# oneapi-src/ishmem

Hardware: AMD Instinct MI355X
Metric: GiB/s device-resident float32 sum-reduce at 1/2/4/8 PEs vs HBM+xGMI roofline (higher is better)
Workload: dtype f32

## Files before the change

### ishmem_amd/csrc/kernels.h

```cpp
#pragma once
#include <hip/hip_runtime.h>
#include <stddef.h>
#include <stdint.h>

#include "types.h"

namespace ishmemi {

constexpr int kMaxPes = 16;
constexpr int kMaxBlocks = 1024;
constexpr int kPhases = 4;
constexpr int kPhaseStart = 0, kPhaseMid = 1, kPhaseEnd = 2, kPhaseSync = 3;
constexpr size_t kFlagWordsPerTeam = (size_t) kPhases * kMaxBlocks * kMaxPes;
constexpr size_t kTeamFlagBytes = kFlagWordsPerTeam * 4 + 256;
constexpr int kBlock = 256;
constexpr int kUnroll = 4;
constexpr int kFaninBlock = 64;
constexpr int kFaninMaxGrid = (int) ((1ull << 31) / kFaninBlock);

constexpr int kEpWords = 16;
constexpr int kLineWords = 16;
constexpr int kEpReplicas = 64;
constexpr int kEpRepLine = 1, kEpShardLine = kEpRepLine + kEpReplicas, kEpShards = 8;
constexpr int kEpTopLine = kEpShardLine + kEpShards;
constexpr int kEpClaimLine = kEpTopLine + 1;
constexpr int kEpTeamWords = kEpClaimLine * kLineWords + kMaxBlocks;
constexpr int kEpEpoch = 0;
constexpr int kEpDone = 1;
constexpr int kEpRsHead = 2;
constexpr int kEpAgHead = 3;
constexpr int kEpStarted = 4;
constexpr int kEpFail = 5;
constexpr int kEpP1Done = 6;
struct ReduceArgs {
    const char *src[kMaxPes];
    const char *dstp[kMaxPes];
    char *dst;
    uint32_t *my_flags;
    uint32_t *peer_flags[kMaxPes];
    uint32_t *err;
    int *ret;
    uint64_t head;
    uint64_t nitems;
    uint64_t tail;
    uint64_t items_per_chunk;
    uint64_t seg_items;
    uint64_t timeout_ticks;
    int oneshot;
    uint32_t *ep_ctr;
    int p, me;
    uint64_t *trace;
};

#ifndef ISHMEMI_LL_TEAM_BYTES
#define ISHMEMI_LL_TEAM_BYTES (8u << 20)
#endif
constexpr size_t kLLTeamBytes = ISHMEMI_LL_TEAM_BYTES;
__host__ __device__ constexpr uint64_t ll_sender_granules(int p)
{
    return ((uint64_t) kLLTeamBytes / 8 / (2 * (uint64_t) (p < 1 ? 1 : p))) & ~uint64_t(127);
}
#ifndef ISHMEMI_LL_PAIRED
#define ISHMEMI_LL_PAIRED 0
#endif
__host__ __device__ constexpr uint64_t ll_granule(uint64_t item, int h)
{
// ... 67 lines not shown
constexpr int kRealignMaxGrid = (int) ((1ull << 31) / kRealignBlock);
#ifndef ISHMEMI_RS_REALIGN_BLOCK
#define ISHMEMI_RS_REALIGN_BLOCK 64
#endif
constexpr int kRsRealignBlock = ISHMEMI_RS_REALIGN_BLOCK;
#ifndef ISHMEMI_REALIGN_PEEL
#define ISHMEMI_REALIGN_PEEL 256
#endif
constexpr uint64_t kRealignPeel = ISHMEMI_REALIGN_PEEL;

struct FaninArgs {
    const char *src[kMaxFanin];
    char *dst;
    uint64_t head, nitems, tail;
    int nsrc;
    int realign;
    uint32_t shift[kMaxFanin];
    uint64_t total;
};

struct PhaseArgs {
    const char *src[kMaxPes];
    const char *dstp[kMaxPes];
    char *dst;
    uint64_t head, nitems, tail;
    uint64_t items_per_chunk;
    uint32_t elem;
    int p, me;
    int peer_nt;
    uint32_t shift;
    uint64_t total;
    int whole;
    int xcd_group;
};
hipError_t launch_rs_phase(int op, int dt, const PhaseArgs &a, hipStream_t s);
hipError_t launch_ag_phase(const PhaseArgs &a, hipStream_t s);

hipError_t launch_allreduce(int op, int dt, bool vec, const ReduceArgs &a, int grid,
                            hipStream_t s);
hipError_t launch_fanin(int op, int dt, bool vec, const FaninArgs &a, int grid, hipStream_t s);
hipError_t launch_team_sync(const ReduceArgs &a, hipStream_t s);
hipError_t launch_pull_probe(const FaninArgs &a, int policy, hipStream_t s);
void set_device_share(int share);
int device_share();
constexpr int kWaitSlotsDefault = 16;
void set_wait_slots(int slots);
int wait_slots();
void set_realign_grid_cap(int cap);
int realign_grid_cap();
void set_collect_realign(int on);
int collect_realign();
void set_phase_unaligned(int on);
int phase_unaligned();
hipError_t launch_occupy(int grid, uint64_t usec, hipStream_t s);
hipError_t launch_produce_u32(uint32_t *dst, const uint32_t *a, const uint32_t *b, uint64_t n, hipStream_t s);

struct RmaArgs {
    char *dst;
    const char *src;
    uint64_t head, nitems, tail;
};
hipError_t launch_rma_copy(const RmaArgs &a, bool put, int max_blocks, hipStream_t s);
hipError_t launch_read_all_u32(uint32_t *out, const uint32_t *p, uint64_t n, int grid, hipStream_t s);

}
```

### ishmem_amd/csrc/kernels_impl.h

```cpp
#pragma once
#include <algorithm>
#include <map>
#include <mutex>
#include <type_traits>

#include "kernels.h"

namespace ishmemi {
namespace {

constexpr int kSysCoherent = 17;
constexpr int kNonTemporal = 2;
constexpr uint64_t kTile = (uint64_t) kBlock * kUnroll;
#ifndef ISHMEMI_AR_OCC
#define ISHMEMI_AR_OCC 4
#endif


template <typename T>
struct alignas(16) Vec {
    T e[16 / sizeof(T)];
};

template <typename T>
// ... 786 lines not shown
    if (i0 + tid < a.nitems) wt_store(make_rsrc(uniform_ptr(a.dst + wo)), tid * 16u, acc);
}

template <typename T, int OP, int NS>
__global__ __launch_bounds__(kRealignBlock) void fanin_realign_kernel(FaninArgs a)
{
    static_assert(NS == 1 || NS == 2, "realigned fan-in: 1 or 2 sources");
    __shared__ u32x4 edge[NS][kRealignWaves + 1];
    const uint32_t tid = threadIdx.x;
    const uint64_t stride = (uint64_t) gridDim.x * kRealignBlock;
    const uint64_t first = (uint64_t) blockIdx.x * kRealignBlock;
    if (stride >= a.nitems) {
        if (first < a.nitems) fanin_realign_block<T, OP, NS>(a, edge, first);
    } else {
        for (uint64_t i0 = first; i0 < a.nitems; i0 += stride) {
            fanin_realign_block<T, OP, NS>(a, edge, i0);
            __syncthreads();
        }
    }
    if (blockIdx.x == 0) {
        const uint64_t tail_off = a.head + a.nitems * (16 / sizeof(T));
        for (int pass = 0; pass < 2; ++pass) {
            const uint64_t cnt = pass == 0 ? a.head : a.tail;
            for (uint64_t t = tid; t < cnt; t += kRealignBlock) {
                const uint64_t e = pass == 0 ? t : tail_off + t;
                T acc = ((const T *) a.src[0])[e];
                if constexpr (NS == 2) acc = op1<T, OP>(acc, ((const T *) a.src[1])[e]);
                ((T *) a.dst)[e] = acc;
            }
        }
    }
}

template <typename T, int OP, int P, bool NT, int R>
__device__ __forceinline__ void rs_phase_item(const PhaseArgs &a, uint64_t wb, bool valid)
{
    using Item = Vec<T>;
    const uint32_t off = threadIdx.x * 16u;
    Item x[P];
#pragma unroll
    for (int k = 0; k < P; ++k) {
        const int j = (R + k) % P;
        if (!valid) continue;
        if (NT || j == a.me) x[k] = bload<Item>(make_rsrc(uniform_ptr(a.src[j] + wb)), off);
        else x[k] = cload<Item>(make_rsrc(uniform_ptr(a.src[j] + wb)), off);
    }
    Item acc = x[(P - R) % P];
#pragma unroll
    for (int j = 1; j < P; ++j) acc = op1<T, OP>(acc, x[(j - R + P) % P]);
    if (valid) wt_store(make_rsrc(uniform_ptr(a.dst + wb)), off, acc);
}

template <typename T, int OP, int P, bool NT, int R = 0>
__device__ __forceinline__ void rs_phase_dispatch(const PhaseArgs &a, int rot, uint64_t wb, bool valid)
{
    if constexpr (R == P - 1) {
        rs_phase_item<T, OP, P, NT, R>(a, wb, valid);
    } else {
        if (rot == R) rs_phase_item<T, OP, P, NT, R>(a, wb, valid);
        else rs_phase_dispatch<T, OP, P, NT, R + 1>(a, rot, wb, valid);
    }
}

template <typename T, int OP>
__device__ __forceinline__ void rs_phase_item_any(const PhaseArgs &a, uint64_t wb, bool valid)
{
    using Item = Vec<T>;
    if (!valid) return;
    const uint32_t off = threadIdx.x * 16u;
    Item acc;
    for (int j = 0; j < a.p; ++j) {
        Item x;
        if (j == a.me || a.peer_nt) x = nt_load((const Item *) (a.src[j] + wb + off));
        else x = cload<Item>(make_rsrc(uniform_ptr(a.src[j] + wb)), off);
        acc = j == 0 ? x : op1<T, OP>(acc, x);
    }
    wt_store(make_rsrc(uniform_ptr(a.dst + wb)), off, acc);
}

template <typename T, int OP>
__device__ __forceinline__ void rs_phase_edges(const PhaseArgs &a)
{
    const int p = a.p, me = a.me;
    if (blockIdx.x == 0) {
        const int tid = threadIdx.x;
        const uint64_t tail_off = a.head + a.nitems * (16 / sizeof(T));
        for (int region = 0; region < 2; ++region) {
            const bool owner = a.whole || (region == 0 ? me == 0 : me == p - 1);
            const uint64_t cnt = region == 0 ? a.head : a.tail;
            if (!owner || (uint64_t) tid >= cnt) continue;
            const uint64_t rbase = (region == 0 ? 0 : tail_off) * sizeof(T);
            const uint32_t off = (uint32_t) (tid * sizeof(T));
            T acc = T();
            for (int j = 0; j < p; ++j) {
                T x;
                if (j == me) x = ((const T *) (a.src[j] + rbase))[tid];
                else x = cload<T>(make_rsrc(uniform_ptr(a.src[j] + rbase)), off);
                acc = (j == 0) ? x : op1<T, OP>(acc, x);
            }
            wt_store(make_rsrc(uniform_ptr(a.dst + rbase)), off, acc);
        }
    }
}

__device__ __forceinline__ uint64_t xcd_grouped_block(uint64_t b, uint64_t grid)
{
    if (b >= (grid & ~63ull)) return b;
    return (b & ~63ull) | ((b & 7) << 3) | ((b >> 3) & 7);
}

template <typename T, int OP, int P>
__global__ __launch_bounds__(kFaninBlock) void rs_phase_kernel(PhaseArgs a)
{
    const int me = a.me;
    const uint64_t cs = a.whole ? 0 : min((uint64_t) me * a.items_per_chunk, a.nitems);
    const uint64_t ce = a.whole ? a.nitems : min(cs + a.items_per_chunk, a.nitems);
    const uint64_t head_bytes = a.head * sizeof(T);
    const uint64_t stride = (uint64_t) gridDim.x * kFaninBlock;
    const uint64_t blk = a.shift && a.xcd_group ? xcd_grouped_block(blockIdx.x, gridDim.x) : blockIdx.x;
    auto body = [&](auto nt) {
        for (uint64_t i0 = cs + blk * kFaninBlock; i0 < ce; i0 += stride) {
            const bool valid = i0 + threadIdx.x < ce;
            const uint64_t wb = head_bytes + i0 * 16;
            if constexpr (P > 0) rs_phase_dispatch<T, OP, P, decltype(nt)::value>(a, (int) ((i0 / kFaninBlock) % P), wb, valid);
            else rs_phase_item_any<T, OP>(a, wb, valid);
        }
    };
    if (a.peer_nt) {
        body(std::true_type{});
    } else {
        body(std::false_type{});
    }
    rs_phase_edges<T, OP>(a);
}

template <typename T, int OP, int BS, int G>
__device__ __forceinline__ void rs_realign_block(const PhaseArgs &a, u32x4 (*edge)[BS / 64 + 1], uint64_t i0, uint64_t ce)
{
    const int p = a.p, me = a.me;
    const uint32_t tid = threadIdx.x;
    const uint64_t wb = a.head * sizeof(T) + i0 * 16;
    Vec<T> acc;
    for (int g0 = 0; g0 < p; g0 += G) {
        if (g0) __syncthreads();
        u32x4 A[G], B[G];
#pragma unroll
        for (int k = 0; k < G; ++k) {
            const int j = g0 + k;
            if (j >= p) break;
            if (j == me || a.peer_nt) realign_issue<kNonTemporal, BS>(a.src[j], a.shift, a.total, wb, edge[k], A[k], B[k]);
            else realign_issue<kSysCoherent, BS>(a.src[j], a.shift, a.total, wb, edge[k], A[k], B[k]);
        }
        __syncthreads();
#pragma unroll
        for (int k = 0; k < G; ++k) {
            const int j = g0 + k;
            if (j >= p) break;
            const Vec<T> x = __builtin_bit_cast(Vec<T>, realign_finish(edge[k], A[k], B[k], a.shift));
            acc = j == 0 ? x : op1<T, OP>(acc, x);
        }
    }
    if (i0 + tid < ce) wt_store(make_rsrc(uniform_ptr(a.dst + wb)), tid * 16u, acc);
}

template <typename T, int OP>
__global__ __launch_bounds__(kRsRealignBlock) void rs_phase_realign_kernel(PhaseArgs a)
{
    constexpr int BS = kRsRealignBlock, G = 4;
    __shared__ u32x4 edge[G][BS / 64 + 1];
    const uint64_t cs = a.whole ? 0 : min((uint64_t) a.me * a.items_per_chunk, a.nitems);
    const uint64_t ce = a.whole ? a.nitems : min(cs + a.items_per_chunk, a.nitems);
    const uint64_t stride = (uint64_t) gridDim.x * BS;
    const uint64_t first = cs + (uint64_t) blockIdx.x * BS;
    if (cs + stride >= ce) {
        if (first < ce) rs_realign_block<T, OP, BS, G>(a, edge, first, ce);
    } else {
        for (uint64_t i0 = first; i0 < ce; i0 += stride) {
            rs_realign_block<T, OP, BS, G>(a, edge, i0, ce);
            __syncthreads();
        }
    }
    rs_phase_edges<T, OP>(a);
}

__global__ __launch_bounds__(kFaninBlock) void ag_phase_kernel(PhaseArgs a)
{
    const int p = a.p, me = a.me;
    const uint64_t head_bytes = a.head * a.elem;
    const uint64_t peers = (uint64_t) (p - 1);
    const uint64_t blocks = (a.items_per_chunk + kFaninBlock - 1) / kFaninBlock;
    const uint64_t work = peers * blocks;
    const uint32_t off = threadIdx.x * 16u;
    for (uint64_t w = blockIdx.x; w < work; w += gridDim.x) {
        const int j = (me + 1 + (int) (w % peers)) % p;
        const uint64_t js = min((uint64_t) j * a.items_per_chunk, a.nitems);
        const uint64_t je = min(js + a.items_per_chunk, a.nitems);
        const uint64_t i0 = js + (w / peers) * kFaninBlock;
        if (i0 + threadIdx.x < je) {
            const uint64_t wb = head_bytes + i0 * 16;
            const u32x4 x = a.peer_nt ? nt_load((const u32x4 *) (a.dstp[j] + wb + off))
                                      : cload<u32x4>(make_rsrc(uniform_ptr(a.dstp[j] + wb)), off);
            wt_store(make_rsrc(uniform_ptr(a.dst + wb)), off, x);
        }
    }
    if (blockIdx.x == 0) {
        const uint32_t tid = threadIdx.x;
        const uint64_t tail_b = (uint64_t) a.tail * a.elem;
        const uint64_t tail_base = head_bytes + a.nitems * 16;
        if (me != 0 && tid < head_bytes)
            a.dst[tid] = (char) cload<uint8_t>(make_rsrc(uniform_ptr(a.dstp[0])), tid);
        if (me != p - 1 && tid < tail_b)
            a.dst[tail_base + tid] = (char) cload<uint8_t>(make_rsrc(uniform_ptr(a.dstp[p - 1] + tail_base)), tid);
    }
}

template <typename K>
int phase_grid(K, uint64_t items)
{
    const uint64_t g = (items + kFaninBlock - 1) / kFaninBlock;
    return (int) std::max<uint64_t>(1, std::min<uint64_t>(g, (uint64_t) kFaninMaxGrid));
}

template <typename T, int OP>
hipError_t rs_phase_t(const PhaseArgs &a, hipStream_t s)
{
    const uint64_t cs = a.whole ? 0 : std::min((uint64_t) a.me * a.items_per_chunk, a.nitems);
    const uint64_t len = a.whole ? a.nitems : std::min(cs + a.items_per_chunk, a.nitems) - cs;
    auto go = [&](auto kernel) {
        hipLaunchKernelGGL(kernel, dim3(phase_grid(kernel, len)), dim3(kFaninBlock), 0, s, a);
    };
    if (a.shift && !phase_unaligned()) {
        uint64_t g = std::max<uint64_t>(1, std::min<uint64_t>((len + kRsRealignBlock - 1) / kRsRealignBlock,
                                                              (1ull << 31) / kRsRealignBlock));
        if (realign_grid_cap() > 0) g = std::min<uint64_t>(g, (uint64_t) realign_grid_cap());
        hipLaunchKernelGGL((rs_phase_realign_kernel<T, OP>), dim3((unsigned) g), dim3(kRsRealignBlock), 0, s, a);
    } else if (a.p == 2) go(rs_phase_kernel<T, OP, 2>);
    else if (a.p == 4) go(rs_phase_kernel<T, OP, 4>);
    else if (a.p == 8) go(rs_phase_kernel<T, OP, 8>);
    else go(rs_phase_kernel<T, OP, 0>);
    return hipGetLastError();
}

template <typename T, int OP>
__device__ __forceinline__ uint64_t fold8(uint64_t acc, uint64_t x)
{
    constexpr int K = 8 / sizeof(T);
    struct alignas(8) W {
        T e[K];
    };
    W a = __builtin_bit_cast(W, acc), b = __builtin_bit_cast(W, x);
#pragma unroll
    for (int i = 0; i < K; ++i) a.e[i] = op1<T, OP>(a.e[i], b.e[i]);
    return __builtin_bit_cast(uint64_t, a);
}

__device__ __forceinline__ uint64_t ll_load(const char *p, uint64_t valid)
{
    if (valid == 8) {
        if (((uintptr_t) p & 7) == 0) return *(const uint64_t *) p;
        if (((uintptr_t) p & 3) == 0)
            return (uint64_t) ((const uint32_t *) p)[0] | ((uint64_t) ((const uint32_t *) p)[1] << 32);
    }
    uint64_t mine = 0;
    for (uint32_t k = 0; k < (uint32_t) valid; ++k) mine |= (uint64_t) (uint8_t) p[k] << (8 * k);
    return mine;
}

__device__ __forceinline__ void ll_store(char *p, uint64_t valid, uint64_t v)
// ... 59 lines not shown
                        __hip_atomic_fetch_or(a.err, 1u << 4, __ATOMIC_RELAXED, __HIP_MEMORY_SCOPE_SYSTEM);
                        break;
                    }
                    __builtin_amdgcn_s_sleep(1);
                }
                x = (h0 & 0xffffffffull) | (h1 << 32);
            }
            if (a.mode == kLLCollect || a2a) ll_store(a.dst + (uint64_t) j * a.nbytes + off, valid, x);
            else if (bcast) { if (j == a.root) ll_store(a.dst + off, valid, x); }
            else if (j <= last) acc = (j == 0) ? x : fold8<T, OP>(acc, x);
        }
        if (ok && a.mode != kLLCollect && !a2a && !bcast) ll_store(a.dst + off, valid, acc);
    }
    if (!ok && a.ret) __hip_atomic_fetch_or(a.ret, 1, __ATOMIC_RELAXED, __HIP_MEMORY_SCOPE_SYSTEM);
    kernel_epoch_done(a, ep);
}

inline int resident_blocks_of(const void *kernel);

template <typename T, int OP>
hipError_t ll_t(const LLArgs &a, hipStream_t s)
{
    const uint64_t nitems = (a.nbytes + 7) / 8;
    const uint64_t want = std::max<uint64_t>(1, (nitems + kBlock - 1) / kBlock);
    const int grid = (int) std::min<uint64_t>(want, (uint64_t) resident_blocks_of((const void *) ll_kernel<T, OP>));
    hipLaunchKernelGGL((ll_kernel<T, OP>), dim3(grid), dim3(kBlock), 0, s, a);
    return hipGetLastError();
}

__global__ __launch_bounds__(kBlock) void team_sync_kernel(ReduceArgs a)
{
    const uint32_t ep = kernel_epoch(a);
    const bool ok = pe_barrier(a, ep, kPhaseSync, 0);
    if (threadIdx.x == 0 && !ok && a.ret)
        __hip_atomic_fetch_or(a.ret, 1, __ATOMIC_RELAXED, __HIP_MEMORY_SCOPE_SYSTEM);
    kernel_epoch_done(a, ep);
}

template <int OP, typename S, typename U>
using Canon = std::conditional_t<(OP == ISHMEMI_OP_MAX || OP == ISHMEMI_OP_MIN), S, U>;

inline int resident_blocks_of(const void *kernel)
{
    static std::mutex mu;
    static std::map<const void *, int> cache;
    static int cus = 0;
    std::lock_guard<std::mutex> lk(mu);
    if (cus <= 0) {
        int dev = 0;
        (void) hipGetDevice(&dev);
        if (hipDeviceGetAttribute(&cus, hipDeviceAttributeMultiprocessorCount, dev) != hipSuccess) {
            (void) hipGetLastError();
            cus = 1;
        }
    }
    int per = 0;
    auto it = cache.find(kernel);
    if (it != cache.end()) {
        per = it->second;
    } else {
        if (hipOccupancyMaxActiveBlocksPerMultiprocessor(&per, kernel, kBlock, 0) != hipSuccess) {
            (void) hipGetLastError();
            per = 1;
        }
        per = std::max(per, 1);
        cache[kernel] = per;
    }
    const long long slots = (long long) device_share() * wait_slots();
// ... 97 lines not shown
```

### ishmem_amd/csrc/runtime.cpp

```cpp
#include <hip/hip_runtime.h>
#include <stdio.h>
#include <stdlib.h>
#include <string.h>
#include <strings.h>
#include <stdint.h>
#include <errno.h>
#include <sys/prctl.h>
#include <unistd.h>

#include <algorithm>
#include <chrono>
#include <limits>
#include <map>
#include <mutex>
#include <string>
#include <vector>

#include "bootstrap.h"
#include "kernels.h"
#include "types.h"

namespace ishmemi {
namespace {

// ... 181 lines not shown
long long wait_slots_floor() { return std::max<long long>(1, env_ll("GPU_MAX_HW_QUEUES", 4)); }

struct Team {
    bool valid = false;
    int start = 0, stride = 1, size = 1;
    int my_idx = -1;
    int num_contexts = 0;
    bool colocated = true;
};

struct TeamMem {
    uint32_t *flags[kMaxPes] = {};
    uint64_t *ring[kMaxPes] = {};
    int pool_idx = -1;
    char *fold_scratch = nullptr;
    size_t fold_scratch_bytes = 0;
};

struct PoolBlock {
    uint32_t *ptr = nullptr;
    hipIpcMemHandle_t handle{};
    bool in_use = false;
};

constexpr long long kPhasedOff = std::numeric_limits<long long>::max();
constexpr long long kPhasedDefault = 4ll << 20;

struct PeRecord {
    int32_t pe, pid, device, flags_kind;
    int32_t flags_kind_requested;
    char pci_bus[32];
    uint64_t heap_size;
    int64_t max_blocks, ll_max_bytes, oneshot_p2, phased_min;
    uint64_t staging_bytes;
    int64_t staging_slots;
    int64_t xgmi_ll_max, xgmi_fold_max;
    hipIpcMemHandle_t heap_handle;
    hipIpcMemHandle_t flags_handle;
};

struct State {
    std::mutex mu;
    bool initialized = false;
    int pe = 0, npes = 1, device = 0;
    ShmBootstrap boot;

    char *heap = nullptr;
    size_t heap_size = 0;
    std::map<size_t, size_t> free_list;
    std::map<size_t, size_t> used;
    char *peer_heap[kMaxPes] = {};

    uint32_t *flags = nullptr;
    int flags_kind = 0;
    uint32_t *peer_flags[kMaxPes] = {};
    int dev_id[kMaxPes] = {};
    TeamMem tmem[kMaxTeams];
    int teams_max = kTeamsMaxDefault;
    size_t team_block_bytes = 0;
    std::vector<PoolBlock> team_pool;
    std::map<std::pair<int, uint32_t>, void *> peer_pool;
    uint32_t *err_host = nullptr;
    uint32_t *err_dev = nullptr;
    uint64_t *exch_host = nullptr, *exch_dev = nullptr;
    uint32_t *done_host = nullptr, *done_dev = nullptr;
    uint32_t done_seq = 0;
    int block_spin = 2;
    ishmemi_c_device_ctx_t *dctx = nullptr;
    uint32_t *dev_epochs = nullptr;
    uint32_t *kern_ep = nullptr;

    char *team_scratch = nullptr;
    char *count_slots = nullptr;
    char *staging = nullptr;
    size_t staging_bytes = 0;
    hipStream_t copy_in = nullptr, copy_out = nullptr;
    hipStream_t rma_stream = nullptr;
    hipEvent_t rma_ev = nullptr;
    bool rma_pending = false;
    hipStream_t last_stream = nullptr;
    bool last_stream_set = false;
    bool stream_order = false;
    long long oneshot_p2 = 32ll << 20;
    long long phased_min = kPhasedDefault;
    hipEvent_t order_ev = nullptr;
    hipEvent_t staging_ev = nullptr;
    bool staging_used = false;
    int staging_slots = kStagingSlotsDefault;
    int staged_copy_kernel = 0;
    bool test_flags_unavailable = false;
    int phased_peer_nt = 0;
    int ar_shifted = 1;
    int rs_xcd = 1;
    int direct_p2 = 1;
    int direct_max_pes = 4;
    int direct_inplace = 1;
    long long xgmi_ll_max = -1, xgmi_fold_max = -1;
    double xgmi_link_bps = 76.8e9;
    hipEvent_t ev_in[kMaxStagingSlots] = {}, ev_red[kMaxStagingSlots] = {}, ev_out[kMaxStagingSlots] = {};

    Team teams[kMaxTeams];
    int max_blocks = kMaxBlocks;
    long long ll_max_bytes = (long long) kLLDefaultBytes;
    long long timeout_ms = 60000;
    int debug = 0;
    int error_count = 0;
    uint64_t *trace = nullptr;
    bool phase_events = false, phase_recorded = false;
    hipEvent_t phase_ev[6] = {};
    double init_us[8] = {};
};

const char *const kInitPhase[8] = {"hip", "heap", "flags", "bootstrap", "ipc_heap", "ipc_flags", "teams", "total"};

State &S()
{
    static State s;
    return s;
}

struct CtxSlots {
    std::mutex mu;
    std::vector<const void *> shadows;
};
// ... 406 lines not shown
    a.ret = ret;
    a.trace = s.trace;
    const void *srcs[1] = {src};
    Plan pl = make_plan(dst, srcs, 1, n, es, t.size, s.max_blocks, 0);
    a.head = pl.head;
    a.nitems = pl.nitems;
    a.tail = pl.tail;
    a.items_per_chunk = pl.items_per_chunk;
    a.seg_items = pl.seg_items;
    const uintptr_t d0 = (uintptr_t) dst, s0 = (uintptr_t) src, nb = n * es;
    const bool realign = !pl.vec && d0 % es == 0 && s0 % es == 0 && nb >= kRealignMinBytes;
    if (realign && (long long) nb < s.phased_min && s.ar_shifted) {
        const void *dsts[1] = {dst};
        pl = make_plan(dst, dsts, 1, n, es, t.size, s.max_blocks, 0);
        a.head = pl.head;
        a.nitems = pl.nitems;
        a.tail = pl.tail;
        a.items_per_chunk = pl.items_per_chunk;
        a.seg_items = pl.seg_items;
    }
    const bool disjoint = d0 + nb <= s0 || s0 + nb <= d0;
    const PathLimits lim = team_limits(s, t);
    const bool fold_size = lim.fold > 0 && (long long) nb <= lim.fold;
    char *scratch = nullptr;
    if (fold_size && d0 == s0 && pl.vec && s.direct_inplace && (uint64_t) t.size * nb <= kInplaceFoldBytes) {
        const TeamMem &m = s.tmem[team];
        if (!m.fold_scratch || m.fold_scratch_bytes < nb + 16)
            return fail("reduce: the team's in-place fold scratch is missing");
        scratch = m.fold_scratch + (d0 & 15);
    }
    const bool inplace_fold = scratch != nullptr;
    const bool direct = (fold_size && disjoint && (pl.vec || realign)) || inplace_fold;
    if ((pl.vec || realign) && (direct || (long long) nb >= s.phased_min)) {
        PhaseArgs ph;
        memset(&ph, 0, sizeof(ph));
        for (int j = 0; j < t.size; ++j) {
            ph.src[j] = a.src[j];
            ph.dstp[j] = a.dstp[j];
        }
        ph.dst = a.dst;
        ph.head = pl.head;
        ph.nitems = pl.nitems;
        ph.tail = pl.tail;
        ph.items_per_chunk = pl.items_per_chunk;
        ph.elem = (uint32_t) es;
        ph.p = t.size;
        ph.me = t.my_idx;
        ph.peer_nt = s.phased_peer_nt;
        ph.whole = direct ? 1 : 0;
        ph.xcd_group = s.rs_xcd && device_share() == 1 ? 1 : 0;
        if (inplace_fold) ph.dst = scratch;
        if (realign) {
            const uint64_t h = std::min<uint64_t>(n, ((16 - d0 % 16) % 16) / es);
            ph.head = h;
            ph.nitems = (n - h) * es / 16;
            ph.tail = n - h - ph.nitems * (16 / es);
            ph.items_per_chunk = items_per_chunk(ph.nitems, t.size);
            ph.shift = (uint32_t) ((s0 + h * es) % 16);
            ph.total = nb;
        }
        const bool ev = s.phase_events && !capturing(st);
        auto mark = [&](int k) -> int {
            if (ev) HIP_TRY(hipEventRecord(s.phase_ev[k], st));
            return 0;
        };
        if (mark(0)) return 1;
        if (team_barrier(s, team, a, st)) return 1;
        if (mark(1)) return 1;
        HIP_TRY(launch_rs_phase(op, dt, ph, st));
        if (mark(2)) return 1;
        if (!direct) {
            if (team_barrier(s, team, a, st)) return 1;
            if (mark(3)) return 1;
            HIP_TRY(launch_ag_phase(ph, st));
        } else if (mark(3)) {
            return 1;
        }
        if (mark(4)) return 1;
        if (team_barrier(s, team, a, st)) return 1;
        if (mark(5)) return 1;
        if (inplace_fold && launch_copy(dst, scratch, nb, st)) return 1;
        s.phase_recorded = s.phase_recorded || ev;
        return 0;
    }
    if (t.size == 2 && (long long) nb <= lim.oneshot && disjoint) {
        a.oneshot = 1;
        a.items_per_chunk = pl.nitems;
        a.seg_items = seg_items(pl.nitems);
        pl.grid = (int) std::max<uint64_t>(
            1, std::min<uint64_t>(nsegs(pl.nitems, a.seg_items), (uint64_t) s.max_blocks));
    }
    HIP_TRY(launch_allreduce(op, dt, pl.vec, a, pl.grid, st));
    return 0;
}

constexpr size_t kPinMinBytes = (size_t) 1 << 20;

bool pageable_host(const void *p)
{
    hipPointerAttribute_t attr;
    if (hipPointerGetAttributes(&attr, p) != hipSuccess) {
        (void) hipGetLastError();
        return true;
    }
// ... 746 lines not shown
    if (env_flag_false("ISHMEM_ENABLE_GPU_IPC") && g_env_error.empty())
        g_env_error = std::string("ISHMEM_ENABLE_GPU_IPC=") + getenv("ISHMEM_ENABLE_GPU_IPC") +
                      " is not supported: ishmem_amd's collectives are IPC-only (peer loads over xGMI from "
                      "IPC-mapped heaps; there is no proxy path)";
    if (env_flag_true("ISHMEM_ENABLE_ACCESSIBLE_HOST_HEAP") && g_env_error.empty())
        g_env_error = std::string("ISHMEM_ENABLE_ACCESSIBLE_HOST_HEAP=") + getenv("ISHMEM_ENABLE_ACCESSIBLE_HOST_HEAP") +
                      " is not supported: the symmetric heap is device memory shared over IPC (host buffers "
                      "are accepted by every call and staged)";
    s.max_blocks = (int) std::min<long long>(kMaxBlocks, std::max<long long>(1, env_ll("ISHMEM_MAX_BLOCKS", kMaxBlocks)));
    s.timeout_ms = std::max<long long>(1, env_ll("ISHMEM_TIMEOUT_MS", 60000));
    s.ll_max_bytes = std::min<long long>((long long) kLLMaxBytes,
                                         std::max<long long>(0, env_bytes("ISHMEM_LL_MAX_BYTES", (long long) kLLDefaultBytes)));
    s.debug = debug_level();
    s.trace = nullptr;
    s.stream_order = env_ll("ISHMEM_STREAM_ORDER", 0) != 0;
    s.oneshot_p2 = std::max<long long>(0, env_bytes("ISHMEM_ONESHOT_P2_MAX_BYTES", 32ll << 20));
    s.phased_min = env_bytes("ISHMEM_PHASED_MIN_BYTES", kPhasedDefault);
    if (s.phased_min < 0) s.phased_min = kPhasedOff;
    s.staging_bytes = (env_size("ISHMEM_STAGING_SIZE", (size_t) 128 << 20) + kHeapAlign - 1) &
                      ~(size_t) (kHeapAlign - 1);
    s.staging_slots = (int) std::min<long long>(kMaxStagingSlots, std::max<long long>(2, env_ll("ISHMEM_STAGING_SLOTS", kStagingSlotsDefault)));
    s.staged_copy_kernel = (int) (env_ll("ISHMEM_STAGED_COPY_KERNEL", kStagedCopyKernelDefault) & 3);
    const size_t heap_request = env_size("ISHMEM_SYMMETRIC_SIZE", (size_t) 4 << 30);
    const int first_kind = (int) std::min<long long>(kFlagsCoarse, std::max<long long>(0, env_ll("ISHMEM_FLAGS_KIND", 0)));
#ifdef ISHMEMI_TEST_HOOKS
    s.test_flags_unavailable = env_ll("ISHMEM_TEST_FLAGS_UNAVAILABLE", 0) != 0;
#else
    for (const char *hook : {"ISHMEM_TEST_FLAGS_UNAVAILABLE", "ISHMEM_TEST_PCI_BUS"})
        if (getenv(hook) && g_env_error.empty())
            g_env_error = std::string(hook) + " is a test hook, honoured only by libishmem_amd_testhooks.so";
#endif
    const bool ep_uncached = env_ll("ISHMEM_EP_UNCACHED", 0) != 0;
    s.phased_peer_nt = env_ll("ISHMEM_PHASED_PEER_NT", 0) != 0;
    s.teams_max = kTeamsMaxDefault;
    if (const char *tm = getenv("ISHMEM_TEAMS_MAX"); tm && *tm) {
        const long long v = env_ll("ISHMEM_TEAMS_MAX", kTeamsMaxDefault);
        if (v < 0 && g_env_error.empty())
            g_env_error = std::string("ISHMEM_TEAMS_MAX='") + tm + "' is not a team count";
        else if (v > kMaxTeams && g_env_error.empty())
            g_env_error = "ISHMEM_TEAMS_MAX=" + std::to_string(v) + ": requested " + std::to_string(v) +
                          " teams, but only " + std::to_string(kMaxTeams) + " are supported";
        s.teams_max = (int) std::min<long long>(kMaxTeams, std::max<long long>(kPredefTeams, v));
    }
    s.xgmi_ll_max = std::max<long long>(-1, env_bytes("ISHMEM_XGMI_LL_MAX_BYTES", -1));
    s.xgmi_fold_max = std::max<long long>(-1, env_bytes("ISHMEM_XGMI_FOLD_MAX_BYTES", -1));
    s.xgmi_link_bps = 76.8e9;
    if (const char *bk = getenv("ISHMEM_BARRIER_KIND"); bk && *bk && strcasecmp(bk, "kernel") != 0 && g_env_error.empty())
        g_env_error = std::string("ISHMEM_BARRIER_KIND='") + bk +
                      "' is not supported: team barriers are the one-workgroup barrier kernel ('kernel')";
    if (!g_env_error.empty()) {
        const std::string e = g_env_error;
        g_env_error.clear();
        return fail("init: " + e);
    }
    warn_unknown_env();

    using clk = std::chrono::steady_clock;
    const auto t_start = clk::now();
    auto t_mark = t_start;
    auto phase_done = [&](int k) {
        const auto now = clk::now();
        s.init_us[k] = std::chrono::duration<double, std::micro>(now - t_mark).count();
        t_mark = now;
        if (s.debug > 1) {
            fprintf(stderr, "[ishmem_amd] PE %d init: %s done (%.1f ms)\n", pe, kInitPhase[k], s.init_us[k] / 1000.0);
            fflush(stderr);
// ... 32 lines not shown
    s.done_host = (uint32_t *) ((char *) s.err_host + kErrDoneOffset);
    s.done_dev = (uint32_t *) ((char *) s.err_dev + kErrDoneOffset);
    s.done_seq = 0;
    HIP_TRY(hipDeviceSynchronize());

    for (int i = 0; i < kMaxPes; ++i) {
        s.peer_heap[i] = nullptr;
        s.peer_flags[i] = nullptr;
    }
    s.peer_heap[pe] = s.heap;
    s.peer_flags[pe] = s.flags;
    for (int i = 0; i < kMaxPes; ++i) s.dev_id[i] = 0;
    phase_done(2);

    if (npes > 1) {
        struct PtracerWindow {
            PtracerWindow() { prctl(PR_SET_PTRACER, PR_SET_PTRACER_ANY, 0, 0, 0); }
            ~PtracerWindow() { prctl(PR_SET_PTRACER, 0, 0, 0, 0); }
        } ptracer_window;
        std::string err;
        if (s.boot.attach(pe, npes, key, (int) std::max<long long>(s.timeout_ms, 10000), err))
            return fail(err);
        PeRecord mine{};
        mine.pe = pe;
        mine.pid = (int32_t) getpid();
        mine.device = s.device;
        mine.flags_kind = s.flags_kind;
        mine.flags_kind_requested = first_kind;
        mine.heap_size = s.heap_size;
        mine.max_blocks = s.max_blocks;
        mine.ll_max_bytes = s.ll_max_bytes;
        mine.oneshot_p2 = s.oneshot_p2;
        mine.phased_min = s.phased_min;
        mine.staging_bytes = s.staging_bytes;
        mine.staging_slots = s.staging_slots;
        mine.xgmi_ll_max = s.xgmi_ll_max;
        mine.xgmi_fold_max = s.xgmi_fold_max;
        if (hipDeviceGetPCIBusId(mine.pci_bus, sizeof(mine.pci_bus), s.device) != hipSuccess) {
            (void) hipGetLastError();
            snprintf(mine.pci_bus, sizeof(mine.pci_bus), "dev%d", s.device);
        }
#ifdef ISHMEMI_TEST_HOOKS
        if (const char *fake = getenv("ISHMEM_TEST_PCI_BUS"))
            snprintf(mine.pci_bus, sizeof(mine.pci_bus), "%s", fake);
#endif
        if (hipError_t e = hipIpcGetMemHandle(&mine.heap_handle, s.heap); e != hipSuccess)
            return fail(std::string("init: hipIpcGetMemHandle of the symmetric heap: ") + hipGetErrorString(e) + ipc_hint());
        mine.flags_handle = flags_handle;
        PeRecord all[kMaxPes];
        if (s.boot.allgather(&mine, all, sizeof(PeRecord), err)) return fail(err);
        phase_done(3);
        for (int j = 0; j < npes; ++j) {
            s.ll_max_bytes = std::min<long long>(s.ll_max_bytes, all[j].ll_max_bytes);
            s.oneshot_p2 = std::min<long long>(s.oneshot_p2, all[j].oneshot_p2);
            s.phased_min = std::max<long long>(s.phased_min, all[j].phased_min);
            s.staging_bytes = std::min<size_t>(s.staging_bytes, all[j].staging_bytes);
            s.staging_slots = (int) std::min<int64_t>(s.staging_slots, all[j].staging_slots);
            if (all[j].xgmi_ll_max >= 0)
                s.xgmi_ll_max = s.xgmi_ll_max < 0 ? all[j].xgmi_ll_max : std::min<long long>(s.xgmi_ll_max, all[j].xgmi_ll_max);
            if (all[j].xgmi_fold_max >= 0)
                s.xgmi_fold_max = s.xgmi_fold_max < 0 ? all[j].xgmi_fold_max
                                                       : std::min<long long>(s.xgmi_fold_max, all[j].xgmi_fold_max);
        }
        int share = 0;
        for (int j = 0; j < npes; ++j)
            share += strncmp(all[j].pci_bus, mine.pci_bus, sizeof(mine.pci_bus)) == 0;
        for (int j = 0; j < npes; ++j) {
            s.dev_id[j] = j;
            for (int k = 0; k < j; ++k)
                if (strncmp(all[j].pci_bus, all[k].pci_bus, sizeof(all[j].pci_bus)) == 0) {
                    s.dev_id[j] = s.dev_id[k];
                    break;
                }
        }
        bool coarse_forced = false;
        for (int j = 0; j < npes; ++j) coarse_forced = coarse_forced || all[j].flags_kind_requested == kFlagsCoarse;
        set_device_share(share);
        for (int j = 0; j < npes; ++j) {
            if (j == pe) continue;
            if (all[j].heap_size != s.heap_size)
                return fail("init: ISHMEM_SYMMETRIC_SIZE differs between PEs");
            if (all[j].device != s.device) {
                int can = 0;
                if (hipDeviceCanAccessPeer(&can, s.device, all[j].device) != hipSuccess || !can)
                    return fail("init: no peer access from device " + std::to_string(s.device) +
                                " to device " + std::to_string(all[j].device) + " (PE " +
                                std::to_string(j) + ")");
                hipError_t e = hipDeviceEnablePeerAccess(all[j].device, 0);
// ... 1209 lines not shown

const char *ishmemi_c_last_error(void) { return g_last_error.c_str(); }

int ishmemi_c_phase_times(float *ms5)
{
    State &s = S();
    if (!ms5) return fail("phase_times: null output");
    if (!s.phase_recorded || !s.phase_ev[0]) return fail("phase_times: no phased reduce recorded (set_param phase_events 1)");
    HIP_TRY(hipEventSynchronize(s.phase_ev[5]));
    for (int k = 0; k < 5; ++k) HIP_TRY(hipEventElapsedTime(&ms5[k], s.phase_ev[k], s.phase_ev[k + 1]));
    return 0;
}

int ishmemi_c_set_param(const char *name, long long value)
{
    State &s = S();
    std::lock_guard<std::mutex> lk(s.mu);
    const std::string n = name ? name : "";
    if (n == "max_blocks") s.max_blocks = (int) std::min<long long>(kMaxBlocks, std::max<long long>(1, value));
    else if (n == "staged_copy_kernel") s.staged_copy_kernel = (int) (value & 3);
    else if (n == "wait_slots") {
        if (value < wait_slots_floor())
            return fail("set_param: wait_slots " + std::to_string(value) + " is below " +
                        std::to_string(wait_slots_floor()) + " (GPU_MAX_HW_QUEUES), see ISHMEM_WAIT_SLOTS");
        set_wait_slots((int) std::min<long long>(1 << 20, value));
    }
    else if (n == "timeout_ms") s.timeout_ms = std::max<long long>(1, value);
    else if (n == "stream_order") s.stream_order = value != 0;
    else if (n == "oneshot_p2_max_bytes") s.oneshot_p2 = std::max<long long>(0, value);
    else if (n == "phased_min_bytes") s.phased_min = value < 0 ? kPhasedOff : value;
    else if (n == "ll_max_bytes") s.ll_max_bytes = std::min<long long>((long long) kLLMaxBytes, std::max<long long>(0, value));
    else if (n == "debug") s.debug = (int) value;
    else if (n == "phased_peer_nt") s.phased_peer_nt = value != 0;
    else if (n == "xgmi_ll_max_bytes") s.xgmi_ll_max = std::max<long long>(-1, value);
    else if (n == "xgmi_fold_max_bytes") s.xgmi_fold_max = std::max<long long>(-1, value);
    else if (n == "xgmi_link_mbps") {
        if (value <= 0) return fail("set_param: xgmi_link_mbps must be positive");
        s.xgmi_link_bps = (double) value * 1e6;
    }
    else if (n == "realign_grid_cap") set_realign_grid_cap((int) std::min<long long>(std::max<long long>(value, 0), 1 << 30));
    else if (n == "collect_realign") set_collect_realign((int) (value != 0));
    else if (n == "ar_shifted") s.ar_shifted = value != 0;
    else if (n == "rs_xcd") s.rs_xcd = value != 0;
    else if (n == "direct_p2") s.direct_p2 = value != 0;
    else if (n == "direct_inplace") s.direct_inplace = value != 0;
    else if (n == "block_spin") s.block_spin = (int) std::min<long long>(std::max<long long>(value, 0), 2);
    else if (n == "direct_max_pes") s.direct_max_pes = (int) std::min<long long>(std::max<long long>(value, 2), kMaxPes);
    else if (n == "phase_unaligned") set_phase_unaligned((int) (value != 0));
    else if (n == "trace_buffer") s.trace = (uint64_t *) (uintptr_t) value;
    else if (n == "phase_events") {
        if (value && !s.phase_ev[0])
            for (hipEvent_t &e : s.phase_ev) HIP_TRY(hipEventCreate(&e));
        s.phase_events = value != 0;
    }
    else return fail("set_param: unknown parameter " + n);
    return 0;
}

long long ishmemi_c_get_param(const char *name)
{
    State &s = S();
    const std::string n = name ? name : "";
    if (n == "max_blocks") return s.max_blocks;
    if (n == "staged_copy_kernel") return s.staged_copy_kernel;
    if (n == "wait_slots") return wait_slots();
    if (n == "timeout_ms") return s.timeout_ms;
    if (n == "stream_order") return s.stream_order ? 1 : 0;
    if (n == "oneshot_p2_max_bytes") return s.oneshot_p2;
    if (n == "phased_min_bytes") return s.phased_min == kPhasedOff ? -1 : s.phased_min;
    if (n == "ll_max_bytes") return s.ll_max_bytes;
    if (n == "ll_capacity_bytes") return (long long) ll_capacity(s.npes);
    if (n == "ll_limit_bytes") return team_limits(s, s.teams[0]).ll;
    if (n == "fold_limit_bytes") return team_limits(s, s.teams[0]).fold;
    if (n == "team_colocated") return s.teams[0].colocated ? 1 : 0;
    if (n == "xgmi_ll_max_bytes") return s.xgmi_ll_max;
    if (n == "xgmi_fold_max_bytes") return s.xgmi_fold_max;
    if (n == "xgmi_link_mbps") return (long long) (s.xgmi_link_bps / 1e6);
    if (n == "teams_max") return s.teams_max;
    if (n == "flag_block_bytes") return s.initialized ? (long long) (kBaseAllocBytes + s.team_block_bytes) : 0;
    if (n == "flag_block_pool_bytes") return (long long) (s.team_pool.size() * kTeamAllocBytes);
    if (n == "flag_block_bytes_round5") return (long long) kRound5FlagBytes;
    for (int k = 0; k < 8; ++k)
        if (n == std::string("init_us_") + kInitPhase[k]) return (long long) s.init_us[k];
    if (n == "debug") return s.debug;
    if (n == "phased_peer_nt") return s.phased_peer_nt;
    if (n == "realign_grid_cap") return realign_grid_cap();
    if (n == "collect_realign") return collect_realign();
    if (n == "ar_shifted") return s.ar_shifted;
    if (n == "rs_xcd") return s.rs_xcd;
    if (n == "direct_p2") return s.direct_p2;
    if (n == "direct_inplace") return s.direct_inplace;
    if (n == "block_spin") return s.block_spin;
    if (n == "direct_max_pes") return s.direct_max_pes;
    if (n == "phase_unaligned") return phase_unaligned();
    if (n == "flags_fine_grained") return s.flags_kind != kFlagsCoarse ? 1 : 0;
    if (n == "flags_kind") return s.flags_kind;
    if (n == "staging_bytes") return (long long) s.staging_bytes;
    if (n == "staging_slots") return s.staging_slots;
    if (n == "heap_bytes") return (long long) s.heap_size;
    if (n == "device_share") return device_share();
    if (n == "launch_words") return (long long) (uintptr_t) s.kern_ep;
    if (n == "cu_count") {
        int dev = 0, cus = 0;
        if (hipGetDevice(&dev) != hipSuccess ||
            hipDeviceGetAttribute(&cus, hipDeviceAttributeMultiprocessorCount, dev) != hipSuccess) {
            (void) hipGetLastError();
            return -1;
        }
        return cus;
    }
    return -1;
}

int ishmemi_c_error_count(void)
{
    State &s = S();
    int pending = 0;
    if (s.err_host)
// ... 46 lines not shown
```

Measured before the change: 3136.

## Push reduced chunks directly to all peers, fusing reduce-scatter with all-gather

In the phased allreduce path, the reduce-scatter kernel can now write each reduced chunk to every peer's destination buffer, rotated by block to spread link traffic. This removes the second team barrier and the separate all-gather kernel launch. A gate word set by the preceding sync kernel turns off all stores if that barrier failed. The cost is more remote writes over xGMI from inside the reduce kernel, with no separate gather step. The behaviour is on by default and can be disabled through an env var or parameter.

Result: no change. 3134 (-0.1%).

```diff
diff --git a/ishmem_amd/csrc/kernels.h b/ishmem_amd/csrc/kernels.h
--- a/ishmem_amd/csrc/kernels.h
+++ b/ishmem_amd/csrc/kernels.h
@@ -32,6 +32,7 @@
 constexpr int kEpStarted = 4;
 constexpr int kEpFail = 5;
 constexpr int kEpP1Done = 6;
+constexpr int kEpSyncFail = kEpTopLine * kLineWords + 1;
 struct ReduceArgs {
     const char *src[kMaxPes];
     const char *dstp[kMaxPes];
@@ -165,6 +166,8 @@
     uint64_t total;
     int whole;
     int xcd_group;
+    int push;
+    const uint32_t *gate;
 };
 hipError_t launch_rs_phase(int op, int dt, const PhaseArgs &a, hipStream_t s);
 hipError_t launch_ag_phase(const PhaseArgs &a, hipStream_t s);
diff --git a/ishmem_amd/csrc/kernels_impl.h b/ishmem_amd/csrc/kernels_impl.h
--- a/ishmem_amd/csrc/kernels_impl.h
+++ b/ishmem_amd/csrc/kernels_impl.h
@@ -842,8 +842,37 @@
     }
 }
 
+template <typename I>
+__device__ __forceinline__ u32x4 pin16(const I &v)
+{
+    static_assert(sizeof(I) == 16, "pin16: a 16-B item");
+    u32x4 r = __builtin_bit_cast(u32x4, v);
+    asm volatile("" : "+v"(r));
+    return r;
+}
+
+template <typename I>
+__device__ __forceinline__ void phase_store(const PhaseArgs &a, int fan, int rot, uint64_t wb, uint32_t off, const I &v)
+{
+    if (fan == 0) {
+        wt_store(make_rsrc(uniform_ptr(a.dst + wb)), off, v);
+    } else if (fan > 0) {
+        int j = rot;
+        for (int k = 0; k < a.p; ++k) {
+            char *d = j == a.me ? a.dst : const_cast<char *>(a.dstp[j]);
+            wt_store(make_rsrc(uniform_ptr(d + wb)), off, v);
+            j = j + 1 == a.p ? 0 : j + 1;
+        }
+    }
+}
+
+__device__ __forceinline__ int phase_fan(const PhaseArgs &a, uint32_t gate)
+{
+    return !a.push ? 0 : (gate == 0 ? 1 : -1);
+}
+
 template <typename T, int OP, int P, bool NT, int R>
-__device__ __forceinline__ void rs_phase_item(const PhaseArgs &a, uint64_t wb, bool valid)
+__device__ __forceinline__ void rs_phase_item(const PhaseArgs &a, int fan, uint64_t wb, bool valid)
 {
     using Item = Vec<T>;
     const uint32_t off = threadIdx.x * 16u;
@@ -858,22 +887,33 @@
     Item acc = x[(P - R) % P];
 #pragma unroll
     for (int j = 1; j < P; ++j) acc = op1<T, OP>(acc, x[(j - R + P) % P]);
-    if (valid) wt_store(make_rsrc(uniform_ptr(a.dst + wb)), off, acc);
+    if (!valid) return;
+    const u32x4 v = pin16(acc);
+    if (fan == 0) {
+        wt_store(make_rsrc(uniform_ptr(a.dst + wb)), off, v);
+    } else if (fan > 0) {
+#pragma unroll
+        for (int k = 0; k < P; ++k) {
+            const int j = (R + k) % P;
+            char *d = j == a.me ? a.dst : const_cast<char *>(a.dstp[j]);
+            wt_store(make_rsrc(uniform_ptr(d + wb)), off, v);
+        }
+    }
 }
 
 template <typename T, int OP, int P, bool NT, int R = 0>
-__device__ __forceinline__ void rs_phase_dispatch(const PhaseArgs &a, int rot, uint64_t wb, bool valid)
+__device__ __forceinline__ void rs_phase_dispatch(const PhaseArgs &a, int fan, int rot, uint64_t wb, bool valid)
 {
     if constexpr (R == P - 1) {
-        rs_phase_item<T, OP, P, NT, R>(a, wb, valid);
+        rs_phase_item<T, OP, P, NT, R>(a, fan, wb, valid);
     } else {
-        if (rot == R) rs_phase_item<T, OP, P, NT, R>(a, wb, valid);
-        else rs_phase_dispatch<T, OP, P, NT, R + 1>(a, rot, wb, valid);
+        if (rot == R) rs_phase_item<T, OP, P, NT, R>(a, fan, wb, valid);
+        else rs_phase_dispatch<T, OP, P, NT, R + 1>(a, fan, rot, wb, valid);
     }
 }
 
 template <typename T, int OP>
-__device__ __forceinline__ void rs_phase_item_any(const PhaseArgs &a, uint64_t wb, bool valid)
+__device__ __forceinline__ void rs_phase_item_any(const PhaseArgs &a, int fan, int rot, uint64_t wb, bool valid)
 {
     using Item = Vec<T>;
     if (!valid) return;
@@ -885,11 +925,11 @@
         else x = cload<Item>(make_rsrc(uniform_ptr(a.src[j] + wb)), off);
         acc = j == 0 ? x : op1<T, OP>(acc, x);
     }
-    wt_store(make_rsrc(uniform_ptr(a.dst + wb)), off, acc);
+    phase_store(a, fan, rot, wb, off, pin16(acc));
 }
 
 template <typename T, int OP>
-__device__ __forceinline__ void rs_phase_edges(const PhaseArgs &a)
+__device__ __forceinline__ void rs_phase_edges(const PhaseArgs &a, int fan)
 {
     const int p = a.p, me = a.me;
     if (blockIdx.x == 0) {
@@ -908,7 +948,7 @@
                 else x = cload<T>(make_rsrc(uniform_ptr(a.src[j] + rbase)), off);
                 acc = (j == 0) ? x : op1<T, OP>(acc, x);
             }
-            wt_store(make_rsrc(uniform_ptr(a.dst + rbase)), off, acc);
+            phase_store(a, fan, me, rbase, off, acc);
         }
     }
 }
@@ -923,6 +963,7 @@
 __global__ __launch_bounds__(kFaninBlock) void rs_phase_kernel(PhaseArgs a)
 {
     const int me = a.me;
+    const int fan = phase_fan(a, *a.gate);
     const uint64_t cs = a.whole ? 0 : min((uint64_t) me * a.items_per_chunk, a.nitems);
     const uint64_t ce = a.whole ? a.nitems : min(cs + a.items_per_chunk, a.nitems);
     const uint64_t head_bytes = a.head * sizeof(T);
@@ -932,8 +973,8 @@
         for (uint64_t i0 = cs + blk * kFaninBlock; i0 < ce; i0 += stride) {
             const bool valid = i0 + threadIdx.x < ce;
             const uint64_t wb = head_bytes + i0 * 16;
-            if constexpr (P > 0) rs_phase_dispatch<T, OP, P, decltype(nt)::value>(a, (int) ((i0 / kFaninBlock) % P), wb, valid);
-            else rs_phase_item_any<T, OP>(a, wb, valid);
+            if constexpr (P > 0) rs_phase_dispatch<T, OP, P, decltype(nt)::value>(a, fan, (int) ((i0 / kFaninBlock) % P), wb, valid);
+            else rs_phase_item_any<T, OP>(a, fan, (int) ((i0 / kFaninBlock) % (uint64_t) a.p), wb, valid);
         }
     };
     if (a.peer_nt) {
@@ -941,11 +982,11 @@
     } else {
         body(std::false_type{});
     }
-    rs_phase_edges<T, OP>(a);
+    rs_phase_edges<T, OP>(a, fan);
 }
 
 template <typename T, int OP, int BS, int G>
-__device__ __forceinline__ void rs_realign_block(const PhaseArgs &a, u32x4 (*edge)[BS / 64 + 1], uint64_t i0, uint64_t ce)
+__device__ __forceinline__ void rs_realign_block(const PhaseArgs &a, int fan, u32x4 (*edge)[BS / 64 + 1], uint64_t i0, uint64_t ce)
 {
     const int p = a.p, me = a.me;
     const uint32_t tid = threadIdx.x;
@@ -970,27 +1011,28 @@
             acc = j == 0 ? x : op1<T, OP>(acc, x);
         }
     }
-    if (i0 + tid < ce) wt_store(make_rsrc(uniform_ptr(a.dst + wb)), tid * 16u, acc);
-}
-
-template <typename T, int OP>
+    if (i0 + tid < ce) phase_store(a, fan, (int) ((i0 / BS) % (uint64_t) p), wb, tid * 16u, pin16(acc));
+}
+
+template <typename T, int OP, bool PUSH>
 __global__ __launch_bounds__(kRsRealignBlock) void rs_phase_realign_kernel(PhaseArgs a)
 {
     constexpr int BS = kRsRealignBlock, G = 4;
     __shared__ u32x4 edge[G][BS / 64 + 1];
+    const int fan = PUSH ? phase_fan(a, *a.gate) : 0;
     const uint64_t cs = a.whole ? 0 : min((uint64_t) a.me * a.items_per_chunk, a.nitems);
     const uint64_t ce = a.whole ? a.nitems : min(cs + a.items_per_chunk, a.nitems);
     const uint64_t stride = (uint64_t) gridDim.x * BS;
     const uint64_t first = cs + (uint64_t) blockIdx.x * BS;
     if (cs + stride >= ce) {
-        if (first < ce) rs_realign_block<T, OP, BS, G>(a, edge, first, ce);
+        if (first < ce) rs_realign_block<T, OP, BS, G>(a, fan, edge, first, ce);
     } else {
         for (uint64_t i0 = first; i0 < ce; i0 += stride) {
-            rs_realign_block<T, OP, BS, G>(a, edge, i0, ce);
+            rs_realign_block<T, OP, BS, G>(a, fan, edge, i0, ce);
             __syncthreads();
         }
     }
-    rs_phase_edges<T, OP>(a);
+    rs_phase_edges<T, OP>(a, fan);
 }
 
 __global__ __launch_bounds__(kFaninBlock) void ag_phase_kernel(PhaseArgs a)
@@ -1043,7 +1085,8 @@
         uint64_t g = std::max<uint64_t>(1, std::min<uint64_t>((len + kRsRealignBlock - 1) / kRsRealignBlock,
                                                               (1ull << 31) / kRsRealignBlock));
         if (realign_grid_cap() > 0) g = std::min<uint64_t>(g, (uint64_t) realign_grid_cap());
-        hipLaunchKernelGGL((rs_phase_realign_kernel<T, OP>), dim3((unsigned) g), dim3(kRsRealignBlock), 0, s, a);
+        if (a.push) hipLaunchKernelGGL((rs_phase_realign_kernel<T, OP, true>), dim3((unsigned) g), dim3(kRsRealignBlock), 0, s, a);
+        else hipLaunchKernelGGL((rs_phase_realign_kernel<T, OP, false>), dim3((unsigned) g), dim3(kRsRealignBlock), 0, s, a);
     } else if (a.p == 2) go(rs_phase_kernel<T, OP, 2>);
     else if (a.p == 4) go(rs_phase_kernel<T, OP, 4>);
     else if (a.p == 8) go(rs_phase_kernel<T, OP, 8>);
@@ -1169,8 +1212,10 @@
 {
     const uint32_t ep = kernel_epoch(a);
     const bool ok = pe_barrier(a, ep, kPhaseSync, 0);
-    if (threadIdx.x == 0 && !ok && a.ret)
-        __hip_atomic_fetch_or(a.ret, 1, __ATOMIC_RELAXED, __HIP_MEMORY_SCOPE_SYSTEM);
+    if (threadIdx.x == 0) {
+        if (!ok && a.ret) __hip_atomic_fetch_or(a.ret, 1, __ATOMIC_RELAXED, __HIP_MEMORY_SCOPE_SYSTEM);
+        a.ep_ctr[kEpSyncFail] = ok ? 0u : 1u;
+    }
     kernel_epoch_done(a, ep);
 }
 
diff --git a/ishmem_amd/csrc/runtime.cpp b/ishmem_amd/csrc/runtime.cpp
--- a/ishmem_amd/csrc/runtime.cpp
+++ b/ishmem_amd/csrc/runtime.cpp
@@ -237,6 +237,7 @@
     char pci_bus[32];
     uint64_t heap_size;
     int64_t max_blocks, ll_max_bytes, oneshot_p2, phased_min;
+    int64_t phased_push;
     uint64_t staging_bytes;
     int64_t staging_slots;
     int64_t xgmi_ll_max, xgmi_fold_max;
@@ -295,6 +296,7 @@
     int staged_copy_kernel = 0;
     bool test_flags_unavailable = false;
     int phased_peer_nt = 0;
+    int phased_push = 1;
     int ar_shifted = 1;
     int rs_xcd = 1;
     int direct_p2 = 1;
@@ -767,6 +769,7 @@
     const bool inplace_fold = scratch != nullptr;
     const bool direct = (fold_size && disjoint && (pl.vec || realign)) || inplace_fold;
     if ((pl.vec || realign) && (direct || (long long) nb >= s.phased_min)) {
+        const bool push = !direct && s.phased_push && !s.phase_events && (d0 == s0 || disjoint);
         PhaseArgs ph;
         memset(&ph, 0, sizeof(ph));
         for (int j = 0; j < t.size; ++j) {
@@ -783,6 +786,8 @@
         ph.me = t.my_idx;
         ph.peer_nt = s.phased_peer_nt;
         ph.whole = direct ? 1 : 0;
+        ph.push = push ? 1 : 0;
+        ph.gate = a.ep_ctr + kEpSyncFail;
         ph.xcd_group = s.rs_xcd && device_share() == 1 ? 1 : 0;
         if (inplace_fold) ph.dst = scratch;
         if (realign) {
@@ -804,7 +809,7 @@
         if (mark(1)) return 1;
         HIP_TRY(launch_rs_phase(op, dt, ph, st));
         if (mark(2)) return 1;
-        if (!direct) {
+        if (!direct && !push) {
             if (team_barrier(s, team, a, st)) return 1;
             if (mark(3)) return 1;
             HIP_TRY(launch_ag_phase(ph, st));
@@ -1617,6 +1622,7 @@
 #endif
     const bool ep_uncached = env_ll("ISHMEM_EP_UNCACHED", 0) != 0;
     s.phased_peer_nt = env_ll("ISHMEM_PHASED_PEER_NT", 0) != 0;
+    s.phased_push = env_ll("ISHMEM_PHASED_PUSH", 1) != 0;
     s.teams_max = kTeamsMaxDefault;
     if (const char *tm = getenv("ISHMEM_TEAMS_MAX"); tm && *tm) {
         const long long v = env_ll("ISHMEM_TEAMS_MAX", kTeamsMaxDefault);
@@ -1715,6 +1721,7 @@
         mine.ll_max_bytes = s.ll_max_bytes;
         mine.oneshot_p2 = s.oneshot_p2;
         mine.phased_min = s.phased_min;
+        mine.phased_push = s.phased_push;
         mine.staging_bytes = s.staging_bytes;
         mine.staging_slots = s.staging_slots;
         mine.xgmi_ll_max = s.xgmi_ll_max;
@@ -1737,6 +1744,7 @@
             s.ll_max_bytes = std::min<long long>(s.ll_max_bytes, all[j].ll_max_bytes);
             s.oneshot_p2 = std::min<long long>(s.oneshot_p2, all[j].oneshot_p2);
             s.phased_min = std::max<long long>(s.phased_min, all[j].phased_min);
+            s.phased_push = (int) std::min<int64_t>(s.phased_push, all[j].phased_push);
             s.staging_bytes = std::min<size_t>(s.staging_bytes, all[j].staging_bytes);
             s.staging_slots = (int) std::min<int64_t>(s.staging_slots, all[j].staging_slots);
             if (all[j].xgmi_ll_max >= 0)
@@ -3012,6 +3020,7 @@
     else if (n == "ll_max_bytes") s.ll_max_bytes = std::min<long long>((long long) kLLMaxBytes, std::max<long long>(0, value));
     else if (n == "debug") s.debug = (int) value;
     else if (n == "phased_peer_nt") s.phased_peer_nt = value != 0;
+    else if (n == "phased_push") s.phased_push = value != 0;
     else if (n == "xgmi_ll_max_bytes") s.xgmi_ll_max = std::max<long long>(-1, value);
     else if (n == "xgmi_fold_max_bytes") s.xgmi_fold_max = std::max<long long>(-1, value);
     else if (n == "xgmi_link_mbps") {
@@ -3064,6 +3073,7 @@
         if (n == std::string("init_us_") + kInitPhase[k]) return (long long) s.init_us[k];
     if (n == "debug") return s.debug;
     if (n == "phased_peer_nt") return s.phased_peer_nt;
+    if (n == "phased_push") return s.phased_push;
     if (n == "realign_grid_cap") return realign_grid_cap();
     if (n == "collect_realign") return collect_realign();
     if (n == "ar_shifted") return s.ar_shifted;
```
